# EasyVision-Ton/VMG

Hardware: AMD Instinct MI355X
Metric: LR-frames/s (train: forward+loss+backward+AdamW), VMG-REDS-few_levels 4x SR (higher is better)
Workload: dtype bf16; 1 GPU; VMG-REDS-few_levels train step, per-GPU batch 4x7x3x64x64 -> 4x SR (BASELINE configs[1]); global_batch=4, frames_per_clip=7, parallelism=dp1, launch=eager, recompute_chains=False, fp8_chains=False

## Files before the change

vmg_amd/csrc/conv_igemm.hip:

```cpp
#include <stdlib.h>

#include <type_traits>

#include "common.h"

namespace {

constexpr int MAX_ISRC = 32;
constexpr int CBMAX = 160;

__host__ __device__ constexpr int kstg(int ks) { return ks > 1 ? ks : 2; }
__host__ __device__ constexpr int stage_bytes(int ks, int ntb, int cb) { return kstg(ks) * 4 * ntb * 16 * cb; }
__host__ __device__ constexpr int stage_stride(int ks, int ntb, int cb) { return (stage_bytes(ks, ntb, cb) + 4095) / 4096 * 4096; }
__host__ __device__ inline int stages_of(int ks, int ch) {
  const int nb = (ch / 8 + 3) / 4;
  return ks > 1 ? ks * nb : (nb + 1) / 2;
}

struct ConvK {
  const char* src[MAX_ISRC];
  long long src_ps[MAX_ISRC];
  short src_ch[MAX_ISRC];
  short src_nst[MAX_ISRC];
  int src_pixb[MAX_ISRC];
// ... 371 lines not shown
    for (int sl = 0; sl < nst_s; ++sl, ++gst) {
      asm volatile("s_waitcnt vmcnt(0)" ::: "memory");
      __builtin_amdgcn_s_barrier();
      asm volatile("" ::: "memory");
      if (gst + RING - 1 < nstages) issue_w(gst + RING - 1);

      int boff[KSTG];
      if (KS > 1) {
        const int base = ky * (TWH * pixb) + min(4 * cbk + g, CH - 1) * CB;
#pragma unroll
        for (int j = 0; j < KSTG; ++j) boff[j] = base + j * pixb;
        if (++ky == KS) { ky = 0; ++cbk; }
      } else {
#pragma unroll
        for (int j = 0; j < KSTG; ++j) boff[j] = min(4 * (2 * sl + j) + g, CH - 1) * CB;
      }
      const char* wslot = wbuf + (gst % RING) * SS + g * (COB * CB) + px * CB;

      Frag<T> xf[2][MT], wf[2][NTB];
      auto load_frags = [&](int j, int set) {
#pragma unroll
        for (int mt = 0; mt < MT; ++mt) xf[set][mt].load(pixp[mt] + boff[j]);
#pragma unroll
        for (int ct = 0; ct < NTB; ++ct) wf[set][ct].load(wslot + j * (4 * COB * CB) + ct * 16 * CB);
      };
      load_frags(0, 0);
#pragma unroll
      for (int j = 0; j < KSTG; ++j) {
        if (j + 1 < KSTG) load_frags(j + 1, (j + 1) & 1);
#pragma unroll
        for (int ct = 0; ct < NTB; ++ct)
#pragma unroll
          for (int mt = 0; mt < MT; ++mt) acc[ct][mt] = mma(wf[j & 1][ct], xf[j & 1][mt], acc[ct][mt]);
      }
    }
  }
  asm volatile("s_waitcnt vmcnt(0)" ::: "memory");

#pragma unroll
  for (int mt = 0; mt < MT; ++mt) {
    f32x4 r[NTB];
#pragma unroll
    for (int ct = 0; ct < NTB; ++ct) r[ct] = acc[ct][mt];
    conv_epilogue_row<T, KS, NTB>(a, r, wave * MT + mt, TH, cb, nt_real, n, ty, tx, m0, px, g);
  }
}

template <int NTB>
struct EpiLds {
  static constexpr int COB = NTB * 16, C8 = 2 * NTB, PSTR = COB * 4 + 16, NIT = (16 * C8 + 63) / 64;
  static constexpr int BYTES = 16 * PSTR;
};

template <int KS, int NTB>
__device__ __forceinline__ void conv_epilogue_prefetch8(const ConvK& a, int row, int TH, int cb, int n, int ty, int tx, long long m0, int lane,
                                                        bf16x8 (&pre_res)[EpiLds<NTB>::NIT], bf16x8 (&pre_aux)[EpiLds<NTB>::NIT]) {
  using E = EpiLds<NTB>;
  const bf16* res = reinterpret_cast<const bf16*>(a.res);
  const bf16* aux = reinterpret_cast<const bf16*>(a.aux);
#pragma unroll
  for (int it = 0; it < E::NIT; ++it) {
    const int j = it * 64 + lane, pxi = j / E::C8, c8 = j - pxi * E::C8;
    long long pix;
    const bool valid = conv_row_pixel<KS>(a, row, TH, n, ty, tx, m0, pxi & 15, pix);
    const int co = cb * E::COB + c8 * 8;
    if (j < 16 * E::C8 && valid && co < a.Cout) {
      if (res) pre_res[it] = *reinterpret_cast<const bf16x8*>(res + pix * a.res_ps + co);
      if (aux) pre_aux[it] = *reinterpret_cast<const bf16x8*>(aux + pix * a.aux_ps + co);
    }
  }
}

template <int KS, int NTB>
__device__ __forceinline__ void conv_epilogue_lds8(const ConvK& a, const f32x4 (&acc)[NTB], char* stg, int row, int TH, int cb, int n, int ty, int tx,
                                                   long long m0, int lane, const bf16x8 (&pre_res)[EpiLds<NTB>::NIT],
                                                   const bf16x8 (&pre_aux)[EpiLds<NTB>::NIT], const float* lbias) {
  using E = EpiLds<NTB>;
  const int px = lane & 15, g = lane >> 4;
#pragma unroll
  for (int ct = 0; ct < NTB; ++ct) *reinterpret_cast<f32x4*>(stg + px * E::PSTR + (ct * 16 + g * 4) * 4) = acc[ct];
  bf16* out = reinterpret_cast<bf16*>(a.out);
  bf16* out_pre = reinterpret_cast<bf16*>(a.out_pre);
  const float neg = a.act == VMG_ACT_RELU ? 0.f : (a.act == VMG_ACT_LRELU ? a.slope : 1.f);
#pragma unroll
  for (int it = 0; it < E::NIT; ++it) {
    const int j = it * 64 + lane, pxi = j / E::C8, c8 = j - pxi * E::C8;
    long long pix;
    const bool valid = conv_row_pixel<KS>(a, row, TH, n, ty, tx, m0, pxi & 15, pix);
    const int co = cb * E::COB + c8 * 8;
    if (!(j < 16 * E::C8 && valid && co < a.Cout) || VMG_DBG(a, 8)) continue;
    const f32x4 lo = *reinterpret_cast<const f32x4*>(stg + pxi * E::PSTR + c8 * 32);
    const f32x4 hi = *reinterpret_cast<const f32x4*>(stg + pxi * E::PSTR + c8 * 32 + 16);
    float v[8] = {lo[0], lo[1], lo[2], lo[3], hi[0], hi[1], hi[2], hi[3]};
    if (a.bias) {
      const f32x4 b0 = *reinterpret_cast<const f32x4*>(lbias + c8 * 8), b1 = *reinterpret_cast<const f32x4*>(lbias + c8 * 8 + 4);
#pragma unroll
      for (int r = 0; r < 4; ++r) { v[r] += b0[r]; v[4 + r] += b1[r]; }
    }
    if (out_pre) {
      bf16x8 t;
#pragma unroll
      for (int r = 0; r < 8; ++r) t[r] = (bf16)v[r];
      *reinterpret_cast<bf16x8*>(out_pre + pix * a.out_ps + co) = t;
    }
    if (a.act == VMG_ACT_GELU) {
#pragma unroll
      for (int r = 0; r < 8; ++r) v[r] = gelu_erf(v[r]) * a.alpha;
    } else {
#pragma unroll
      for (int r = 0; r < 8; ++r) v[r] = (v[r] > 0.f ? v[r] : v[r] * neg) * a.alpha;
    }
    if (a.aux) {
#pragma unroll
      for (int r = 0; r < 8; ++r) {
        const float u = (float)pre_aux[it][r];
        v[r] *= a.actgrad == 3 ? gelu_erf_grad(u) : (u > 0.f ? 1.f : (a.actgrad == 2 ? a.slope : 0.f));
      }
    }
    if (a.res) {
#pragma unroll
      for (int r = 0; r < 8; ++r) v[r] += (float)pre_res[it][r];
    }
    bf16x8 t;
#pragma unroll
    for (int r = 0; r < 8; ++r) t[r] = (bf16)v[r];
    *reinterpret_cast<bf16x8*>(out + pix * a.out_ps + co) = t;
  }
}

template <typename T, int KS, int NTB>
__global__ __launch_bounds__(256, (NTB <= 3 ? 3 : 2)) void conv_ksplit_kernel(const ConvK a) {
  constexpr int ES = ElemTraits<T>::ES, CB = ElemTraits<T>::CHUNKB;
  constexpr int TH = 4;
  constexpr int TWH = 16 + KS - 1;
  constexpr int COB = NTB * 16;
  constexpr int SS = stage_stride(KS, NTB, CB);
  constexpr int KSB = 4 * COB * CB;
  extern __shared__ __attribute__((aligned(16))) char smem[];
  char* halo = smem;
  char* zslot = smem + a.halo_bytes;
  float* lbias = reinterpret_cast<float*>(zslot + 16);
  if (VMG_DBG(a, 16)) return;

  const int tid = threadIdx.x, lane = tid & 63;
  const int wave = __builtin_amdgcn_readfirstlane(tid >> 6);
  const int px = lane & 15, g = lane >> 4;
  const int cb = blockIdx.y;
  const int nt_real = min(NTB, (a.Cout - cb * COB + 15) >> 4);
  int n = 0, ty = 0, tx = 0;
  long long m0 = 0;
  if (KS > 1) {
    int bid = xcd_remap(blockIdx.x, gridDim.x, a.dbg);
    tx = bid % a.tiles_x;
    int r = bid / a.tiles_x;
    ty = r % a.tiles_y;
    n = r / a.tiles_y;
  } else {
    m0 = (long long)blockIdx.x * 64;
  }
  conv_stamp(a, wave, 0);
  if (tid < 4) reinterpret_cast<int*>(zslot)[tid] = 0;
  const float bias_r = (tid < COB && a.bias && cb * COB + tid < a.Cout) ? a.bias[cb * COB + tid] : 0.f;

  constexpr bool BF = std::is_same<T, bf16>::value;
  const bool vec8 = BF && a.vec8 != 0;
  bf16x8 pre_res[EpiLds<NTB>::NIT], pre_aux[EpiLds<NTB>::NIT];
  if (vec8) conv_epilogue_prefetch8<KS, NTB>(a, wave, TH, cb, n, ty, tx, m0, lane, pre_res, pre_aux);

  f32x4 acc[NTB][4];
#pragma unroll
  for (int ct = 0; ct < NTB; ++ct)
#pragma unroll
    for (int i = 0; i < 4; ++i) acc[ct][i] = f32x4{0.f, 0.f, 0.f, 0.f};

  const char* wlane = a.wpack + (long long)cb * a.nstages * SS + g * (COB * CB) + px * CB;
  int st0 = 0;
  for (int s = 0; s < a.nsrc; ++s) {
    const int ch = a.src_ch[s], pixb = a.src_pixb[s];
    const int CH = ch >> 3, nb = (CH + 3) >> 2;
    if (s > 0) __syncthreads();
    conv_stamp(a, wave, 1);
    stage_halo<T, KS, 1>(a, s, halo, n, ty, tx, m0, tid);
    if (s == 0 && tid < COB) lbias[tid] = bias_r;
    conv_stamp(a, wave, 3);
    __syncthreads();
    conv_stamp(a, wave, 4);

    const int nks = VMG_DBG(a, 32) ? 0 : (KS > 1 ? 9 * nb : nb);
    const int per = ((nks + 3) / 4 + 2) / 3 * 3;
    const int k0 = wave * per;
    const int rowb = TWH * pixb;
    const char* pixp = halo + px * pixb;
    int rowoff[4];
#pragma unroll
    for (int i = 0; i < 4; ++i) rowoff[i] = ((wave + i) & 3) * rowb;

    Frag<T> wf[3][NTB], xf[3][4];
    struct Cur { int k, cbk, ky, kx; long long woff; };
    auto cur_at = [&](int k) {
      Cur c;
      c.k = k;
      const int kc = min(k, nks - 1);
      if (KS > 1) {
        c.cbk = kc / 9;
        const int tap = kc - 9 * c.cbk;
        c.ky = tap / 3;
        c.kx = tap - 3 * c.ky;
        c.woff = (long long)(st0 + c.cbk * 3 + c.ky) * SS + c.kx * KSB;
      } else {
        c.cbk = kc; c.ky = 0; c.kx = 0;
        c.woff = (long long)(st0 + (kc >> 1)) * SS + (kc & 1) * KSB;
      }
      return c;
    };
    auto advance = [&](Cur& c) {
      ++c.k;
      if (c.k < nks) {
        if (KS > 1) {
          c.woff += KSB;
          if (++c.kx == 3) {
            c.kx = 0;
            c.woff += SS - 3 * KSB;
            if (++c.ky == 3) { c.ky = 0; ++c.cbk; }
          }
        } else {
          c.woff += (c.k & 1) ? KSB : SS - KSB;
          c.cbk = c.k;
        }
      }
    };
    Cur cw = cur_at(k0), cx = cw;
    auto load_w = [&](int set) {
      const char* p = wlane + cw.woff;
#pragma unroll
      for (int ct = 0; ct < NTB; ++ct) wf[set][ct].load(p + ct * 16 * CB);
      advance(cw);
    };
    auto load_x = [&](int set) {
      const bool real = cx.k < nks;
      const int boff = (KS > 1 ? cx.ky * rowb + cx.kx * pixb : 0) + min(4 * cx.cbk + g, CH - 1) * CB;
      const char* base = real ? pixp + boff : zslot;
#pragma unroll
      for (int i = 0; i < 4; ++i) xf[set][i].load(base + (real ? rowoff[i] : 0));
      advance(cx);
    };
    auto mfma_set = [&](int set) {
#pragma unroll
      for (int ct = 0; ct < NTB; ++ct)
#pragma unroll
        for (int i = 0; i < 4; ++i) acc[ct][i] = mma(wf[set][ct], xf[set][i], acc[ct][i]);
    };
    if (nks > 0) {
      load_w(0);
      load_w(1);
      load_x(0);
      for (int i = 0; i < per; i += 3) {
        load_w(2);
        load_x(1);
        mfma_set(0);
        load_w(0);
        load_x(2);
        mfma_set(1);
        load_w(1);
        load_x(0);
        mfma_set(2);
      }
    }
    st0 += a.src_nst[s];
  }

  conv_stamp(a, wave, 5);
  __syncthreads();
  char* scratch = smem;
#pragma unroll
  for (int i = 1; i < 4; ++i) {
    const int q = (wave + i) & 3, j = 4 - i;
    char* dst = scratch + ((q * 3 + (j - 1)) * NTB) * 1024 + lane * 16;
#pragma unroll
    for (int ct = 0; ct < NTB; ++ct) *reinterpret_cast<f32x4*>(dst + ct * 1024) = acc[ct][i];
  }
  __syncthreads();
  f32x4 own[NTB];
#pragma unroll
  for (int ct = 0; ct < NTB; ++ct) own[ct] = acc[ct][0];
#pragma unroll
  for (int j = 1; j < 4; ++j) {
    const char* src = scratch + ((wave * 3 + (j - 1)) * NTB) * 1024 + lane * 16;
#pragma unroll
    for (int ct = 0; ct < NTB; ++ct) {
      const f32x4 t = *reinterpret_cast<const f32x4*>(src + ct * 1024);
      own[ct] += t;
    }
  }
  conv_stamp(a, wave, 6);
  if (vec8) {
    static_assert(EpiLds<NTB>::BYTES <= 3 * NTB * 1024, "epilogue staging patch must fit the wave's own scratch slots");
    conv_epilogue_lds8<KS, NTB>(a, own, scratch + (wave * 3 * NTB) * 1024, wave, TH, cb, n, ty, tx, m0, lane, pre_res, pre_aux, lbias);
  } else {
    conv_epilogue_row<T, KS, NTB, false>(a, own, wave, TH, cb, nt_real, n, ty, tx, m0, px, g);
  }
  conv_stamp(a, wave, 7);
}

template <int NTB, int NS = 1>
__global__ __launch_bounds__(256, NS == 1 ? 2 : 1) void linear_wres_kernel(const ConvK a, int ntiles, int tiles_per_wave) {
  using T = bf16;
  constexpr int KS = 1, CB = 16, NKS = 5, NK = NKS * NS, NDMA = NK;
  constexpr int COB = NTB * 16;
  constexpr int SS = stage_stride(KS, NTB, CB);
  constexpr int KSB = 4 * COB * CB;
  constexpr int XBUF = NDMA * 1024;
  constexpr int WAVE_LDS = 2 * XBUF + ((EpiLds<NTB>::BYTES + 1023) & ~1023);
  extern __shared__ __attribute__((aligned(16))) char smem[];
  const int tid = threadIdx.x, lane = tid & 63;
  const int wave = __builtin_amdgcn_readfirstlane(tid >> 6);
  const int px = lane & 15, g = lane >> 4;
  const int cb = blockIdx.y;
  char* xbuf = smem + wave * WAVE_LDS;
  char* patch = xbuf + 2 * XBUF;
  const int CH = a.src_ch[0] >> 3, nb = (CH + 3) >> 2;
  const int vpp = CH * NS;
  const int pixb = vpp * 16;
  const long long ps_b = a.src_ps[0] * 2;
  const int t0 = (blockIdx.x * 4 + wave) * tiles_per_wave, t1 = min(ntiles, t0 + tiles_per_wave);
  if (t0 >= t1) return;

  Frag<T> wres[NK][NTB];
  {
    const char* wlane = a.wpack + (long long)cb * a.nstages * SS + g * (COB * CB) + px * CB;
#pragma unroll
    for (int k = 0; k < NK; ++k) {
      const int sb = k / NKS, kk = k - sb * NKS;
      const int kc = min(kk, nb - 1);
      const char* p = wlane + (long long)(sb * a.src_nst[0] + (kc >> 1)) * SS + (kc & 1) * KSB;
#pragma unroll
      for (int ct = 0; ct < NTB; ++ct) {
        wres[k][ct].load(p + ct * 16 * CB);
        if (kk >= nb) wres[k][ct].v = bf16x8{0, 0, 0, 0, 0, 0, 0, 0};
      }
    }
  }
  int c_off[NDMA];
  int c_row[NDMA];
#pragma unroll
  for (int i = 0; i < NDMA; ++i) {
    const int L = 64 * i + lane;
    const int r = (int)(((float)L + 0.5f) * (1.0f / (float)vpp));
    c_row[i] = L < 16 * vpp ? r : 16;
    c_off[i] = (int)(r * ps_b) + (L - r * vpp) * 16;
  }
  auto issue = [&](int t, int buf) {
    const long long m0 = (long long)t * 16;
    const char* origin = a.src[0] + m0 * ps_b;
    const long long left = a.M - m0;
#pragma unroll
    for (int i = 0; i < NDMA; ++i) {
      const bool ok = c_row[i] < 16 && c_row[i] < left;
      const char* gp = ok ? origin + c_off[i] : reinterpret_cast<const char*>(&g_conv_zero16);
      __builtin_amdgcn_global_load_lds(GLB_PTR(gp), LDS_PTR(xbuf + buf * XBUF + i * 1024), 16, 0, 0);
    }
  };
  int boff[NK];
#pragma unroll
  for (int k = 0; k < NK; ++k) {
    const int sb = k / NKS, kk = k - sb * NKS;
    boff[k] = px * pixb + (sb * CH + min(4 * kk + g, CH - 1)) * CB;
  }

  issue(t0, 0);
  int buf = 0;
  for (int t = t0; t < t1; ++t, buf ^= 1) {
    const long long m0 = (long long)t * 16;
    bf16x8 pre_res[EpiLds<NTB>::NIT], pre_aux[EpiLds<NTB>::NIT];
    conv_epilogue_prefetch8<KS, NTB>(a, 0, 4, cb, 0, 0, 0, m0, lane, pre_res, pre_aux);
    if (t + 1 < t1) {
      issue(t + 1, buf ^ 1);
      asm volatile("s_waitcnt vmcnt(%0)" ::"n"(NDMA) : "memory");
    } else {
      asm volatile("s_waitcnt vmcnt(0)" ::: "memory");
    }
    f32x4 acc[NTB];
#pragma unroll
    for (int ct = 0; ct < NTB; ++ct) acc[ct] = f32x4{0.f, 0.f, 0.f, 0.f};
    const char* xb = xbuf + buf * XBUF;
#pragma unroll
    for (int k = 0; k < NK; ++k) {
      Frag<T> xf;
      xf.load(xb + boff[k]);
#pragma unroll
      for (int ct = 0; ct < NTB; ++ct) acc[ct] = mma(wres[k][ct], xf, acc[ct]);
    }
    conv_epilogue_lds8<KS, NTB>(a, acc, patch, 0, 4, cb, 0, 0, 0, m0, lane, pre_res, pre_aux, a.bias ? a.bias + cb * COB : nullptr);
  }
}

template <int NCT, int NB, bool FULL>
__global__ __launch_bounds__(512, 1) void conv_wstat_kernel(const ConvK a, int ntiles) {
  using T = bf16;
  constexpr int KS = 3, CB = 16, TH = 8, TWH = 18, THH = 10;
  constexpr int COB = NCT * 16, KSB = 4 * COB * CB;
  constexpr int SS = stage_stride(KS, NCT, CB);
  constexpr int NK = 9 * NB, RW = NCT < 2 ? NCT : 2;
  constexpr int PIXB = 144;
  constexpr int HVEC = THH * TWH * 9, NDMA = (HVEC + 63) / 64, HB = NDMA * 1024;
  constexpr int PSTR = COB * 4 + 16, C8 = 2 * NCT, NITEM = 128 * C8;
  extern __shared__ __attribute__((aligned(16))) char smem[];
  const int tid = threadIdx.x, lane = tid & 63;
  const int wave = __builtin_amdgcn_readfirstlane(tid >> 6);
  const int px = lane & 15, g = lane >> 4;
  const int cb = blockIdx.y;
  const int CH = a.src_ch[0] >> 3;
  constexpr int wbytes = 3 * NB * SS;
  char* wl = smem;
  char* halo = smem + wbytes;
  float* lbias = reinterpret_cast<float*>(halo + 2 * HB);
  char* patch = halo + 2 * HB + COB * 4;

  const int per_xcd = gridDim.x >> 3;
  const int xcd = blockIdx.x & 7, local = blockIdx.x >> 3;
  const int band = (ntiles + 7) >> 3;
  const int band0 = xcd * band, band1 = min(ntiles, band0 + band);
  auto tile_of = [&](int it) { return band0 + it * per_xcd + local; };
  auto barrier = [&]() {
    asm volatile("s_waitcnt lgkmcnt(0)" ::: "memory");
    __builtin_amdgcn_s_barrier();
    asm volatile("" ::: "memory");
  };

  {
    const char* wblk = a.wpack + (long long)cb * wbytes;
    for (int i = tid * 16; i < wbytes; i += 512 * 16) *reinterpret_cast<uint4*>(wl + i) = *reinterpret_cast<const uint4*>(wblk + i);
    for (int i = tid; i < COB; i += 512) lbias[i] = (a.bias && cb * COB + i < a.Cout) ? a.bias[cb * COB + i] : 0.f;
  }

  if (wave >= 4) {
    const int h = wave - 4;
    constexpr int NDH = (NDMA + 3) / 4;
    int lpos[NDH], loff[NDH];
    const long long ps_b = a.src_ps[0] * 2;
#pragma unroll
    for (int k = 0; k < NDH; ++k) {
      const int v = 64 * (h + 4 * k) + lane;
      const int p = v / 9, c = v - p * 9;
      const int hy = p / TWH, hx = p - hy * TWH;
      lpos[k] = (v < HVEC && c < CH) ? (hy << 8) | hx : -1;
      loff[k] = (hy * a.W + hx) * (int)ps_b + c * 16;
    }
    int lfast[NDH];
#pragma unroll
    for (int k = 0; k < NDH; ++k) lfast[k] = lpos[k] >= 0 ? loff[k] : 0;
    auto issue_halo = [&](int t, int buf) {
      const int tx = t % a.tiles_x, r = t / a.tiles_x;
      const int ty = r % a.tiles_y, n = r / a.tiles_y;
      const int y0 = ty * TH - 1, x0 = tx * 16 - 1;
      const char* origin = a.src[0] + (((long long)n * a.H + y0) * a.W + x0) * ps_b;
      char* dst = halo + buf * HB;
      if (VMG_DBG(a, 1)) return;
      if (y0 >= 0 && x0 >= 0 && y0 + THH <= a.H && x0 + TWH <= a.W) {
#pragma unroll
        for (int k = 0; k < NDH; ++k) {
          if (h + 4 * k >= NDMA) break;
          glds16_asm_s(origin, lfast[k], dst + (h + 4 * k) * 1024);
        }
        return;
      }
#pragma unroll
      for (int k = 0; k < NDH; ++k) {
        if (h + 4 * k >= NDMA) break;
        const bool ok = lpos[k] >= 0 && (unsigned)(y0 + (lpos[k] >> 8)) < (unsigned)a.H && (unsigned)(x0 + (lpos[k] & 255)) < (unsigned)a.W;
        const char* gp = ok ? origin + loff[k] : reinterpret_cast<const char*>(&g_conv_zero16);
        glds16_asm(gp, dst + (h + 4 * k) * 1024);
      }
    };
    bf16* out = reinterpret_cast<bf16*>(a.out);
    bf16* out_pre = FULL ? reinterpret_cast<bf16*>(a.out_pre) : nullptr;
    const bf16* res = FULL ? reinterpret_cast<const bf16*>(a.res) : nullptr;
    const bf16* aux = FULL ? reinterpret_cast<const bf16*>(a.aux) : nullptr;
    const float neg = a.act == VMG_ACT_RELU ? 0.f : (a.act == VMG_ACT_LRELU ? a.slope : 1.f);
    int ipos[NCT], ipatch[NCT], ico[NCT];
#pragma unroll
    for (int i = 0; i < NCT; ++i) {
      const int j = 64 * h + lane + 256 * i;
      const int p = j / C8, c8 = j - p * C8;
      ipos[i] = ((p >> 4) << 8) | (p & 15);
      ipatch[i] = p * PSTR + c8 * 32;
      ico[i] = c8 * 8;
    }
    const int nstore = NCT * (out_pre ? 2 : 1);
    int ioff[NCT];
    float ibias[NCT][8];
#pragma unroll
    for (int i = 0; i < NCT; ++i) {
      ioff[i] = (((ipos[i] >> 8) * a.W + (ipos[i] & 255)) * (int)a.out_ps + ico[i]) * 2;
#pragma unroll
      for (int q = 0; q < 8; ++q) ibias[i][q] = (a.bias && cb * COB + ico[i] + q < a.Cout) ? a.bias[cb * COB + ico[i] + q] : 0.f;
    }

    if (tile_of(0) < band1) issue_halo(tile_of(0), 0);
    asm volatile("s_waitcnt vmcnt(0)" ::: "memory");
    for (int it = 0;; ++it) {
      barrier();
      const bool more = tile_of(it) < band1;
      if (more && tile_of(it + 1) < band1) issue_halo(tile_of(it + 1), (it + 1) & 1);
      if (it > 0 && !VMG_DBG(a, 64)) {
        const int t = tile_of(it - 1);
        const int tx = t % a.tiles_x, r = t / a.tiles_x;
        const int ty = r % a.tiles_y, n = r / a.tiles_y;
        const long long pix0 = ((long long)n * a.H + ty * TH) * a.W + tx * 16;
        if (!FULL && ty * TH + TH <= a.H && tx * 16 + 16 <= a.W && cb * COB + COB <= a.Cout && !VMG_DBG(a, 8)) {
          char* obase = reinterpret_cast<char*>(out + pix0 * a.out_ps + cb * COB);
#pragma unroll
          for (int i = 0; i < NCT; ++i) {
            const f32x4 lo = *reinterpret_cast<const f32x4*>(patch + ipatch[i]);
            const f32x4 hi = *reinterpret_cast<const f32x4*>(patch + ipatch[i] + 16);
            float v[8] = {lo[0], lo[1], lo[2], lo[3], hi[0], hi[1], hi[2], hi[3]};
            bf16x8 tq;
#pragma unroll
            for (int q = 0; q < 8; ++q) {
              if (a.bias) v[q] += ibias[i][q];
              v[q] = (v[q] > 0.f ? v[q] : v[q] * neg) * a.alpha;
              tq[q] = (bf16)v[q];
            }
            *reinterpret_cast<bf16x8*>(obase + ioff[i]) = tq;
          }
        } else
#pragma unroll
        for (int i = 0; i < NCT; ++i) {
          const int y = ty * TH + (ipos[i] >> 8), x = tx * 16 + (ipos[i] & 255);
          const int co = cb * COB + ico[i];
          const bool valid = y < a.H && x < a.W && co < a.Cout && !VMG_DBG(a, 8);
          const long long pix = valid ? pix0 + (long long)(ipos[i] >> 8) * a.W + (ipos[i] & 255) : 0;
          const f32x4 lo = *reinterpret_cast<const f32x4*>(patch + ipatch[i]);
          const f32x4 hi = *reinterpret_cast<const f32x4*>(patch + ipatch[i] + 16);
          float v[8] = {lo[0], lo[1], lo[2], lo[3], hi[0], hi[1], hi[2], hi[3]};
          if (a.bias) {
            const f32x4 b0 = *reinterpret_cast<const f32x4*>(lbias + ico[i]), b1 = *reinterpret_cast<const f32x4*>(lbias + ico[i] + 4);
#pragma unroll
            for (int q = 0; q < 4; ++q) { v[q] += b0[q]; v[4 + q] += b1[q]; }
          }
          const int cov = valid ? co : 0;
          if (out_pre) {
            bf16x8 tq;
#pragma unroll
            for (int q = 0; q < 8; ++q) tq[q] = (bf16)v[q];
            bf16* dstp = valid ? out_pre + pix * a.out_ps + co : reinterpret_cast<bf16*>(&g_wstat_trash);
            *reinterpret_cast<bf16x8*>(dstp) = tq;
          }
          if (FULL && a.act == VMG_ACT_GELU) {
#pragma unroll
            for (int q = 0; q < 8; ++q) v[q] = gelu_erf(v[q]) * a.alpha;
          } else {
#pragma unroll
            for (int q = 0; q < 8; ++q) v[q] = (v[q] > 0.f ? v[q] : v[q] * neg) * a.alpha;
          }
          if (aux) {
            const bf16x8 au = *reinterpret_cast<const bf16x8*>(aux + pix * a.aux_ps + cov);
#pragma unroll
            for (int q = 0; q < 8; ++q) {
              const float u = (float)au[q];
              v[q] *= a.actgrad == 3 ? gelu_erf_grad(u) : (u > 0.f ? 1.f : (a.actgrad == 2 ? a.slope : 0.f));
            }
          }
          if (res) {
            const bf16x8 rv = *reinterpret_cast<const bf16x8*>(res + pix * a.res_ps + cov);
#pragma unroll
            for (int q = 0; q < 8; ++q) v[q] += (float)rv[q];
          }
          bf16x8 tq;
#pragma unroll
          for (int q = 0; q < 8; ++q) tq[q] = (bf16)v[q];
          bf16* dst = valid ? out + pix * a.out_ps + co : reinterpret_cast<bf16*>(&g_wstat_trash);
          *reinterpret_cast<bf16x8*>(dst) = tq;
        }
      }
      if (!more) break;
      barrier();
      if (it > 0 && !VMG_DBG(a, 64)) {
        if (nstore == NCT) asm volatile("s_waitcnt vmcnt(%0)" ::"n"(NCT) : "memory");
        else asm volatile("s_waitcnt vmcnt(%0)" ::"n"(2 * NCT) : "memory");
      } else {
        asm volatile("s_waitcnt vmcnt(0)" ::: "memory");
      }
    }
    return;
  }

  barrier();
  Frag<T> wreg[NK][RW];
  const char* wlane = wl + g * (COB * CB) + px * CB;
#pragma unroll
  for (int j = 0; j < NK; ++j)
#pragma unroll
    for (int ct = 0; ct < RW; ++ct) wreg[j][ct].load(wlane + (j / 3) * SS + (j % 3) * KSB + ct * 16 * CB);
  for (int it = 0;; ++it) {
    const int t = tile_of(it);
    if (t >= band1) break;
    const int buf = it & 1;
    f32x4 acc[2][NCT];
#pragma unroll
    for (int mt = 0; mt < 2; ++mt)
#pragma unroll
      for (int ct = 0; ct < NCT; ++ct) acc[mt][ct] = f32x4{0.f, 0.f, 0.f, 0.f};
    const char* hb = halo + buf * HB + ((2 * wave) * TWH + px) * PIXB;
    if (!VMG_DBG(a, 32)) {
      Frag<T> xf[2][2], wf[2][NCT > RW ? NCT - RW : 1];
      auto load_frags = [&](int j, int set) {
        const int cbk = j / 9, tap = j - cbk * 9, ky = tap / 3, kx = tap - ky * 3;
        const char* xc = hb + min(4 * cbk + g, CH - 1) * CB;
#pragma unroll
        for (int mt = 0; mt < 2; ++mt) xf[set][mt].load(xc + ((mt + ky) * TWH + kx) * PIXB);
#pragma unroll
        for (int ct = RW; ct < NCT; ++ct) wf[set][ct - RW].load(wlane + (j / 3) * SS + (j % 3) * KSB + ct * 16 * CB);
      };
      load_frags(0, 0);
#pragma unroll
      for (int j = 0; j < NK; ++j) {
        if (j + 1 < NK) load_frags(j + 1, (j + 1) & 1);
#pragma unroll
        for (int ct = 0; ct < NCT; ++ct)
#pragma unroll
          for (int mt = 0; mt < 2; ++mt) acc[mt][ct] = mma(ct < RW ? wreg[j][ct < RW ? ct : 0] : wf[j & 1][ct >= RW ? ct - RW : 0], xf[j & 1][mt], acc[mt][ct]);
      }
    }
    barrier();
#pragma unroll
    for (int mt = 0; mt < 2; ++mt)
#pragma unroll
      for (int ct = 0; ct < NCT; ++ct) *reinterpret_cast<f32x4*>(patch + ((2 * wave + mt) * 16 + px) * PSTR + (ct * 16 + g * 4) * 4) = acc[mt][ct];
    barrier();
  }
}

template <int NCT>
struct WsGeo {
  static constexpr int COB = NCT * 16;
  static constexpr int KSB = COB * 64;
  static constexpr int STG = 3 * KSB;
  static constexpr int TH = 8, TWH = 18, THH = 10;
  static constexpr int NLW = 3;
  static constexpr int THREADS = (4 + NLW) * 64;
  static constexpr int NIT = EpiLds<NCT>::NIT;
};
__host__ __device__ inline int ws_rem_ksteps(int R) { return R == 0 ? 0 : (R == 1 ? 3 : (R == 2 ? 6 : 9)); }
__host__ __device__ inline int ws_ksteps(int CH) { return 9 * (CH / 4) + ws_rem_ksteps(CH % 4); }
__host__ __device__ inline void ws_slot(int CH, int j, int g, int& tap, int& chunk) {
  const int nfull = CH / 4, R = CH % 4;
  if (j < 9 * nfull) { tap = j % 9; chunk = 4 * (j / 9) + g; return; }
  const int jr = j - 9 * nfull;
  if (R == 1) { tap = 4 * jr + g; chunk = 4 * nfull; }
  else if (R == 2) { tap = 2 * jr + (g >> 1); chunk = 4 * nfull + (g & 1); }
  else { tap = (g == 3) ? -1 : jr; chunk = 4 * nfull + (g == 3 ? 0 : g); }
  if (tap > 8) tap = -1;
}

__device__ __forceinline__ void ws_stamp(const ConvK& a, int wave, int slot) {
#ifdef VMG_DIAG
  if (a.stamps && slot < 32) {
    const unsigned long long t = __builtin_amdgcn_s_memrealtime();
    if ((threadIdx.x & 63) == 0) a.stamps[((size_t)(blockIdx.y * gridDim.x + blockIdx.x) * 8 + wave) * 32 + slot] = t;
  }
#endif
}

template <int NCT>
struct WsItems {
  static constexpr int C8 = 2 * NCT, TOTAL = 128 * C8, THREADS = WsGeo<NCT>::THREADS, NIT = (TOTAL + THREADS - 1) / THREADS;
  static constexpr int PSTR = NCT * 64 + 16;
  __device__ static __forceinline__ void decode(int j, int& pxl, int& c8) {
    pxl = NCT == 9 ? (j * 3641) >> 16 : (NCT == 7 ? (j * 4682) >> 16 : (NCT == 8 ? j >> 4 : (j * 10923) >> 16));
    c8 = j - pxl * C8;
  }
};

template <int NCT>
__global__ __launch_bounds__(WsGeo<NCT>::THREADS, (NCT <= 3 ? 4 : 2)) void conv_ws_kernel(const ConvK a) {
  using G = WsGeo<NCT>;
  using I = WsItems<NCT>;
  using T = bf16;
  constexpr int COB = G::COB, KSB = G::KSB, STG = G::STG;
  static_assert(128 * I::PSTR <= 3 * STG, "the epilogue patch must fit the ring");
  extern __shared__ __attribute__((aligned(16))) char smem[];
  char* halo = smem;
  char* ring = smem + a.halo_bytes;
  const int R = a.ring;
  float* lbias = reinterpret_cast<float*>(ring + R * STG);
  const int tid = threadIdx.x, lane = tid & 63;
  const int wave = __builtin_amdgcn_readfirstlane(tid >> 6);
  const int cb = blockIdx.y;
  const int bid = xcd_remap(blockIdx.x, gridDim.x, 0);
  const int tx = bid % a.tiles_x;
  const int rr = bid / a.tiles_x;
  const int ty = rr % a.tiles_y, n = rr / a.tiles_y;
  const int nstages = a.nstages;
  ws_stamp(a, wave, 0);

  auto issue_halo = [&](int s, int first, int step, auto hidden) {
// ... 721 lines not shown
  using G = WsGeo<NCT>;
  ConvK kk = k;
  kk.ring = NCT <= 3 ? 3 : ((k.halo_bytes + 4 * G::STG + G::COB * 4 <= 160 * 1024) ? 4 : 3);
  const int lds = k.halo_bytes + kk.ring * G::STG + G::COB * 4;
  VMG_CHECK(lds <= 160 * 1024, "conv (weight-streaming): LDS request %d B exceeds 160 KiB", lds);
  auto fn = conv_ws_kernel<NCT>;
  static bool attr_set[VMG_MAX_DEVICES] = {};
  const int dev = vmg_current_device();
  if (!attr_set[dev]) {
    (void)hipFuncSetAttribute(reinterpret_cast<const void*>(fn), hipFuncAttributeMaxDynamicSharedMemorySize, 160 * 1024);
    attr_set[dev] = true;
  }
  const long long nblk = (long long)k.N * k.tiles_y * k.tiles_x;
  VMG_CHECK(nblk > 0 && nblk < (1ll << 31), "conv: bad grid %lld", nblk);
  const bool prof = (k.nsrc == 1 && k.src_ch[0] == k.Cout && (k.Cout == 144 || k.Cout == 112)) && vmg_prof_before(VMG_PROF_CONV3X3, k.M, st);
  hipLaunchKernelGGL(fn, dim3((unsigned)nblk, ncb), dim3(G::THREADS), lds, st, kk);
  if (prof) vmg_prof_after(st);
  VMG_LAUNCH_CHECK();
  return 0;
}

}

#ifdef VMG_DIAG
static unsigned long long* g_conv_stamps = nullptr;
#endif
extern "C" int vmg_conv_debug_stamps(void* buf) {
#ifdef VMG_DIAG
  g_conv_stamps = (unsigned long long*)buf;
  return 0;
#else
  (void)buf;
  vmg_set_error("conv_debug_stamps: this library was built without -DVMG_DIAG (VMG_DIAG=1 python -m vmg_amd.build)");
  return -1;
#endif
}

extern "C" int64_t vmg_conv_pack_bytes(int dtype, int ks, int on, int nsrc, const int* src_ch, int cout_tiles) {
  short xoff[MAX_ISRC], xch[MAX_ISRC];
  const int n = expand_sources(nsrc, nullptr, src_ch, xoff, xch, nullptr);
  if (n < 0 || cout_tiles <= 0 || (ks != 1 && ks != 3 && ks != 7)) return -1;
  int64_t nst = 0;
  for (int s = 0; s < n; ++s) nst += stages_of(ks, xch[s]);
  const int cob = cout_tiles * 16;
  const int ncb = (on + cob - 1) / cob;
  return (int64_t)ncb * nst * stage_stride(ks, cout_tiles, dtype == VMG_BF16 ? 16 : 32);
}

static int fill_pack_std(PackK& p, long long& total, int dtype, const float* w, int O, int I, int ks, int o0, int on, int nsrc, const int* src_off,
                         const int* src_ch, int transpose_flip, int cout_tiles, void* packed) {
  VMG_CHECK(w && packed, "conv_pack: null pointer");
  VMG_CHECK(ks == 1 || ks == 3 || ks == 7, "conv_pack: ks must be 1, 3 or 7");
  VMG_CHECK(dtype == VMG_F32 || dtype == VMG_BF16, "conv_pack: bad dtype");
  VMG_CHECK(nsrc >= 1 && nsrc <= 4, "conv_pack: nsrc must be 1..4");
  VMG_CHECK(!(transpose_flip & 1) || nsrc == 1, "conv_pack: data-gradient packing takes one K slice");
  VMG_CHECK(cout_tiles >= 1 && cout_tiles <= 9, "conv_pack: cout_tiles must be 1..9");
  memset(&p, 0, sizeof(p));
  const int n = expand_sources(nsrc, src_off, src_ch, p.src_off, p.src_ch, nullptr);
  VMG_CHECK(n > 0, "conv_pack: channel slices must be multiples of 8 (and split into <= %d blocks)", MAX_ISRC);
  int st = 0;
  for (int s = 0; s < n; ++s) {
    p.src_st0[s] = (short)st;
    p.src_nst[s] = (short)stages_of(ks, p.src_ch[s]);
    st += p.src_nst[s];
  }
  const int groups = (transpose_flip >> 8) > 1 ? (transpose_flip >> 8) : 1;
  transpose_flip &= 1;
  VMG_CHECK(groups == 1 || (O % groups == 0), "conv_pack: output channels must divide into the groups");
  const int Id = I * groups;
  const int kdim = transpose_flip ? O : Id, odim = transpose_flip ? Id : O;
  for (int s = 0; s < n; ++s) VMG_CHECK(p.src_off[s] >= 0 && p.src_off[s] + p.src_ch[s] <= kdim, "conv_pack: K slice out of range");
  VMG_CHECK(o0 >= 0 && o0 + on <= odim, "conv_pack: output slice out of range");
  p.w = w; p.out = (char*)packed; p.O = O; p.I = I; p.ks = ks; p.o0 = o0; p.on = on; p.nsrc = n;
  p.transpose_flip = transpose_flip; p.groups = groups; p.cob = cout_tiles * 16; p.ncb = (on + p.cob - 1) / p.cob; p.nstages = st;
  const int es = dtype == VMG_BF16 ? 2 : 4;
  p.ss_elems = stage_stride(ks, cout_tiles, es * 8) / es;
  total = (long long)p.ncb * p.nstages * p.ss_elems;
  VMG_CHECK(total < (1ll << 31), "conv_pack: pack of %lld elements (the index arithmetic is 32-bit)", total);
  if (ks == 3 && groups == 1 && (transpose_flip || (uintptr_t)w % 16 == 0) && (transpose_flip || I % 4 == 0)) {
    int nblk = 0;
    for (int s = 0; s < n; ++s) nblk += ((p.src_ch[s] >> 3) + 3) >> 2;
    p.fast3 = 1;
    p.units = (long long)p.ncb * nblk * 4 * p.cob + (long long)p.ncb * p.nstages * (p.ss_elems / 8 - 3 * 4 * p.cob);
  }
  return 0;
}

extern "C" int vmg_conv_pack(int dtype, const float* w, int O, int I, int ks, int o0, int on, int nsrc, const int* src_off,
                             const int* src_ch, int transpose_flip, int cout_tiles, void* packed, void* stream) {
  PackK p;
  long long total = 0;
  const int rc = fill_pack_std(p, total, dtype, w, O, I, ks, o0, on, nsrc, src_off, src_ch, transpose_flip, cout_tiles, packed);
  if (rc) return rc;
  if (p.fast3) {
    const int fb = (int)((p.units + 255) / 256 > 4096 ? 4096 : (p.units + 255) / 256);
    if (dtype == VMG_BF16) hipLaunchKernelGGL((pack3_kernel<bf16, false>), dim3(fb), dim3(256), 0, (hipStream_t)stream, p);
    else hipLaunchKernelGGL((pack3_kernel<float, false>), dim3(fb), dim3(256), 0, (hipStream_t)stream, p);
    VMG_LAUNCH_CHECK();
    return 0;
  }
  const int blocks = (int)((total + 255) / 256 > 4096 ? 4096 : (total + 255) / 256);
  if (dtype == VMG_BF16) hipLaunchKernelGGL(conv_pack_kernel<bf16>, dim3(blocks), dim3(256), 0, (hipStream_t)stream, p);
  else hipLaunchKernelGGL(conv_pack_kernel<float>, dim3(blocks), dim3(256), 0, (hipStream_t)stream, p);
  VMG_LAUNCH_CHECK();
  return 0;
}

static int ws_plan(int nsrc, const int* src_off, const int* src_ch, PackK& p) {
  const int n = expand_sources(nsrc, src_off, src_ch, p.src_off, p.src_ch, nullptr);
  if (n <= 0) return -1;
  int st = 0;
  for (int s = 0; s < n; ++s) {
    p.src_st0[s] = (short)st;
    p.src_nst[s] = (short)(ws_ksteps(p.src_ch[s] >> 3) / 3);
    st += p.src_nst[s];
  }
  p.nsrc = n;
  p.nstages = st;
  return n;
}

extern "C" int64_t vmg_convws_pack_bytes(int on, int nsrc, const int* src_ch, int cout_tiles) {
  PackK p;
  memset(&p, 0, sizeof(p));
  if (cout_tiles <= 0 || cout_tiles > 9 || on <= 0 || nsrc < 1 || nsrc > 4 || ws_plan(nsrc, nullptr, src_ch, p) <= 0) return -1;
  const int cob = cout_tiles * 16;
  return (int64_t)cdiv(on, cob) * p.nstages * 3 * (int64_t)cob * 64;
}

static int fill_pack_ws(PackK& p, long long& total, const float* w, int O, int I, int o0, int on, int nsrc, const int* src_off, const int* src_ch,
                        int transpose_flip, int cout_tiles, void* packed) {
  VMG_CHECK(w && packed, "convws_pack: null pointer");
  VMG_CHECK(cout_tiles == 3 || cout_tiles == 7 || cout_tiles == 8 || cout_tiles == 9, "convws_pack: cout_tiles must be 3, 7, 8 or 9");
  VMG_CHECK(nsrc >= 1 && nsrc <= 4, "convws_pack: nsrc must be 1..4");
  VMG_CHECK(!(transpose_flip & 1) || nsrc == 1, "convws_pack: data-gradient packing takes one K slice");
  const int groups = (transpose_flip >> 8) > 1 ? (transpose_flip >> 8) : 1;
  transpose_flip &= 1;
  VMG_CHECK(groups == 1 || (O % groups == 0), "convws_pack: output channels must divide into the groups");
  memset(&p, 0, sizeof(p));
  VMG_CHECK(ws_plan(nsrc, src_off, src_ch, p) > 0, "convws_pack: channel slices must be multiples of 8 (and split into <= %d blocks)", MAX_ISRC);
  const int Id = I * groups;
  const int kdim = transpose_flip ? O : Id, odim = transpose_flip ? Id : O;
  for (int s = 0; s < p.nsrc; ++s) VMG_CHECK(p.src_off[s] >= 0 && p.src_off[s] + p.src_ch[s] <= kdim, "convws_pack: K slice out of range");
  VMG_CHECK(o0 >= 0 && on > 0 && o0 + on <= odim, "convws_pack: output slice out of range");
  p.w = w; p.out = (char*)packed; p.O = O; p.I = I; p.ks = 3; p.o0 = o0; p.on = on; p.transpose_flip = transpose_flip; p.groups = groups;
  p.cob = cout_tiles * 16; p.ncb = cdiv(on, p.cob);
  total = (long long)p.ncb * p.nstages * 3 * 4 * p.cob * 8;
  VMG_CHECK(total < (1ll << 31), "convws_pack: pack of %lld elements (the index arithmetic is 32-bit)", total);
  bool rem_ok = true;
  for (int s = 0; s < p.nsrc; ++s) rem_ok = rem_ok && (((p.src_ch[s] >> 3) & 3) == 0 || ((p.src_ch[s] >> 3) & 3) == 2);
  if (groups == 1 && rem_ok && (transpose_flip || ((uintptr_t)w % 16 == 0 && I % 4 == 0))) {
    int nblk = 0;
    for (int s = 0; s < p.nsrc; ++s) nblk += ((p.src_ch[s] >> 3) + 3) >> 2;
    p.fast3 = 1;
    p.units = (long long)p.ncb * nblk * 4 * p.cob;
  }
  return 0;
}

extern "C" int vmg_convws_pack(const float* w, int O, int I, int o0, int on, int nsrc, const int* src_off, const int* src_ch,
                               int transpose_flip, int cout_tiles, void* packed, void* stream) {
  PackK p;
  long long total = 0;
  const int rc = fill_pack_ws(p, total, w, O, I, o0, on, nsrc, src_off, src_ch, transpose_flip, cout_tiles, packed);
  if (rc) return rc;
  if (p.fast3) {
    const int fb = (int)((p.units + 255) / 256 > 4096 ? 4096 : (p.units + 255) / 256);
    hipLaunchKernelGGL((pack3_kernel<bf16, true>), dim3(fb), dim3(256), 0, (hipStream_t)stream, p);
    VMG_LAUNCH_CHECK();
    return 0;
  }
  const int blocks = (int)((total + 255) / 256 > 4096 ? 4096 : (total + 255) / 256);
  hipLaunchKernelGGL(convws_pack_kernel, dim3(blocks), dim3(256), 0, (hipStream_t)stream, p);
  VMG_LAUNCH_CHECK();
  return 0;
}

extern "C" int vmg_pack_entry_bytes(void) { return (int)sizeof(PackEntry); }

extern "C" int vmg_pack_entry(void* entry, int kind, int dtype, const float* w, int O, int I, int ks, int o0, int on, int nsrc, const int* src_off,
                              const int* src_ch, int transpose_flip, int cout_tiles, void* packed, int blk0) {
  VMG_CHECK(entry && (kind == 0 || kind == 1) && blk0 >= 0, "pack_entry: bad arguments");
  PackEntry e;
  memset(&e, 0, sizeof(e));
  int rc;
  if (kind == 1) {
    VMG_CHECK(ks == 3 && dtype == VMG_BF16, "pack_entry: the weight-streaming layout is bf16 3x3");
    rc = fill_pack_ws(e.p, e.total, w, O, I, o0, on, nsrc, src_off, src_ch, transpose_flip, cout_tiles, packed);
  } else {
    rc = fill_pack_std(e.p, e.total, dtype, w, O, I, ks, o0, on, nsrc, src_off, src_ch, transpose_flip, cout_tiles, packed);
  }
  if (rc) return rc;
  e.kind = kind; e.dtype = dtype; e.blk0 = blk0;
  long long nb = e.p.fast3 ? (e.p.units + 255) / 256 : (e.total + 256LL * 16 - 1) / (256LL * 16);
  e.nblk = (int)(nb < 1 ? 1 : (nb > 64 ? 64 : nb));
  memcpy(entry, &e, sizeof(e));
  return e.nblk;
}

extern "C" int vmg_pack_run(const void* plan_dev, int n, int total_blocks, void* stream) {
  VMG_CHECK(plan_dev && n > 0 && total_blocks > 0, "pack_run: bad arguments");
  static_assert(sizeof(PackEntry) % 4 == 0, "the block-owner table sits behind the entries");
  hipLaunchKernelGGL(pack_batch_kernel, dim3(total_blocks), dim3(256), 0, (hipStream_t)stream, (const PackEntry*)plan_dev, n);
  VMG_LAUNCH_CHECK();
  return 0;
}

extern "C" int vmg_conv_fwd(const vmg_conv_desc* d, void* stream) {
  VMG_CHECK(d != nullptr, "conv_fwd: null descriptor");
  VMG_CHECK(d->ks == 1 || d->ks == 3 || d->ks == 7, "conv_fwd: ks must be 1, 3 or 7");
  VMG_CHECK(d->dtype == VMG_F32 || d->dtype == VMG_BF16, "conv_fwd: bad dtype");
  VMG_CHECK(d->nsrc >= 1 && d->nsrc <= 4, "conv_fwd: nsrc must be 1..4");
  VMG_CHECK(d->N > 0 && d->H > 0 && d->W > 0 && d->Cout > 0, "conv_fwd: bad shape");
  VMG_CHECK(d->packed && d->out, "conv_fwd: null packed weights / output");
  VMG_CHECK(!d->pixel_shuffle || (d->Cout % 4 == 0), "conv_fwd: pixel_shuffle needs Cout %% 4 == 0");
  VMG_CHECK(!(d->actgrad != 0 && d->aux == nullptr), "conv_fwd: actgrad without aux");
  VMG_CHECK(d->deep == VMG_CONV_GENERAL || d->deep == VMG_CONV_KSPLIT || d->deep == VMG_CONV_WS || d->deep == VMG_CONV_LINEAR_WRES ||
                d->deep == VMG_CONV_WSTAT,
            "conv_fwd: unknown kernel route deep = %d", d->deep);
  const int es = d->dtype == VMG_BF16 ? 2 : 4, cbytes = es * 8;
  ConvK k;
  memset(&k, 0, sizeof(k));
  short xoff[MAX_ISRC];
  int parent[MAX_ISRC];
  const int n = expand_sources(d->nsrc, nullptr, d->src_ch, xoff, k.src_ch, parent);
  VMG_CHECK(n > 0, "conv_fwd: source channel counts must be multiples of 8");
  int mt = d->mt;
  if (d->dtype == VMG_F32) mt = 1;
  const long long M = (long long)d->N * d->H * d->W;
  const int ntb = d->cout_tiles;
  VMG_CHECK(ntb > 0, "conv_fwd: cout_tiles must be positive");
  const int ncb = cdiv(d->Cout, ntb * 16);
  if (d->ks == 7) mt = 1;
  if (mt == 0) mt = 1;
  VMG_CHECK(mt == 1 || mt == 2, "conv_fwd: mt must be 1 or 2");
  const int TH = 4 * mt, TWH = 16 + d->ks - 1, THH = TH + d->ks - 1;
  int kt = 0, halo = 0;
  for (int s = 0; s < n; ++s) {
    const int par = parent[s];
    VMG_CHECK(d->src[par] != nullptr, "conv_fwd: null source %d", par);
    VMG_CHECK(d->src_ps[par] >= d->src_ch[par] && (d->src_ps[par] * es) % 16 == 0, "conv_fwd: source pixel stride must be >= channels and 16-byte aligned");
    VMG_CHECK(((uintptr_t)d->src[par]) % 16 == 0, "conv_fwd: source pointer must be 16-byte aligned");
    k.src[s] = (const char*)d->src[par] + (long long)xoff[s] * es;
    k.src_ps[s] = d->src_ps[par];
    k.src_nst[s] = (short)stages_of(d->ks, k.src_ch[s]);
    k.src_pixb[s] = choose_pixb(k.src_ch[s], es, cbytes);
    kt += k.src_nst[s];
    const int hb = THH * TWH * k.src_pixb[s];
    if (hb > halo) halo = hb;
  }
  k.nsrc = n;
  k.wpack = (const char*)d->packed; k.bias = d->bias;
  k.out = (char*)d->out; k.out_ps = d->out_ps; k.out_pre = (char*)d->out_pre;
  k.res = (const char*)d->res; k.res_ps = d->res_ps; k.aux = (const char*)d->aux; k.aux_ps = d->aux_ps;
  k.N = d->N; k.H = d->H; k.W = d->W; k.Cout = d->Cout; k.M = M;
  k.tiles_x = cdiv(d->W, 16); k.tiles_y = cdiv(d->H, TH);
  k.act = d->act; k.slope = d->slope; k.alpha = d->alpha; k.actgrad = d->aux ? d->actgrad : 0; k.ps = d->pixel_shuffle;
#ifdef VMG_DIAG
  {
    const char* e = getenv("VMG_CONV_DBG");
    k.dbg = e ? atoi(e) : 0;
    k.stamps = g_conv_stamps;
  }
#endif
  {
    auto al = [](const void* p) { return ((uintptr_t)p & 15) == 0; };
    k.vec8 = d->dtype == VMG_BF16 && !d->pixel_shuffle && (d->Cout % 16) == 0 && (d->out_ps % 8) == 0 && al(d->out) &&
             (!d->out_pre || al(d->out_pre)) && (!d->res || ((d->res_ps % 8) == 0 && al(d->res))) &&
             (!d->aux || ((d->aux_ps % 8) == 0 && al(d->aux)));
  }
  k.nstages = kt; k.halo_bytes = (halo + 1023) & ~1023;
  VMG_CHECK(d->out_ps >= (d->pixel_shuffle ? d->Cout / 4 : d->Cout), "conv_fwd: out pixel stride too small");
  hipStream_t st = (hipStream_t)stream;
  if (d->deep == VMG_CONV_WS) {
    VMG_CHECK(d->dtype == VMG_BF16 && d->ks == 3 && k.vec8 && (ntb == 3 || ntb == 7 || ntb == 8 || ntb == 9), "conv_fwd: the weight-streaming kernel is bf16 3x3 with 16-byte aligned rows, cout_tiles 3, 7, 8 or 9");
    for (int s = 0; s < n; ++s) VMG_CHECK(k.src_ch[s] % 16 == 0, "conv_fwd: the weight-streaming kernel takes channel blocks that are multiples of 16 (got %d)", k.src_ch[s]);
    int kt3 = 0, halo3 = 0;
    for (int s = 0; s < n; ++s) {
      k.src_pixb[s] = k.src_ch[s] * 2;
      k.src_nst[s] = (short)(ws_ksteps(k.src_ch[s] >> 3) / 3);
      kt3 += k.src_nst[s];
      const int hb = 10 * 18 * k.src_pixb[s];
      if (hb > halo3) halo3 = hb;
    }
    k.nstages = kt3;
    k.halo_bytes = (halo3 + 1023) & ~1023;
    k.tiles_y = cdiv(d->H, 8);
    return ntb == 9 ? launch_ws<9>(k, ncb, st) : (ntb == 7 ? launch_ws<7>(k, ncb, st) : (ntb == 8 ? launch_ws<8>(k, ncb, st) : launch_ws<3>(k, ncb, st)));
  }
  if (d->deep == VMG_CONV_WSTAT && d->dtype == VMG_BF16 && d->ks == 3 && mt == 1 && k.vec8 && n == 1 && (ntb == 1 || ntb == 3 || ntb == 4) && k.src_ch[0] <= 64 && k.src_ch[0] % 8 == 0 &&
      k.src_ps[0] % 8 == 0 && d->W <= 255 * 16 && (long long)d->W * k.src_ps[0] * 2 * 10 < (1ll << 31)) {
    ConvK kk = k;
    kk.tiles_y = cdiv(d->H, 8);
    const int nb = (k.src_ch[0] / 8 + 3) / 4;
    switch (ntb * 2 + (nb - 1)) {
      case 2: return launch_wstat<1, 1>(kk, ncb, st);
      case 3: return launch_wstat<1, 2>(kk, ncb, st);
      case 6: return launch_wstat<3, 1>(kk, ncb, st);
      case 7: return launch_wstat<3, 2>(kk, ncb, st);
      case 8: return launch_wstat<4, 1>(kk, ncb, st);
      case 9: return launch_wstat<4, 2>(kk, ncb, st);
    }
  }
  if (d->deep == VMG_CONV_LINEAR_WRES && d->dtype == VMG_BF16 && d->ks == 1 && k.vec8 && (ntb == 3 || ntb == 5)) {
    if (n == 1 && k.src_ch[0] <= 160 && k.src_pixb[0] == k.src_ch[0] * 2) return ntb == 3 ? launch_linear_wres<3>(k, ncb, st) : launch_linear_wres<5>(k, ncb, st);
    if (n == 2 && ntb == 3 && d->nsrc == 1 && k.src_ch[0] == k.src_ch[1] && k.src_ch[0] <= 160 && k.src[1] == k.src[0] + k.src_ch[0] * 2 &&
        k.src_nst[0] == k.src_nst[1])
      return launch_linear_wres<3, 2>(k, ncb, st);
  }
  if (d->ks == 7) return d->dtype == VMG_BF16 ? dispatch_ks7<bf16>(k, ntb, ncb, st) : dispatch_ks7<float>(k, ntb, ncb, st);
  if (d->deep == VMG_CONV_KSPLIT) {
    VMG_CHECK(d->dtype == VMG_BF16 && mt == 1, "conv_fwd: the k-split variant is bf16, mt = 1");
    return d->ks == 3 ? dispatch_ksplit<bf16, 3>(k, ntb, ncb, k.halo_bytes, st) : dispatch_ksplit<bf16, 1>(k, ntb, ncb, k.halo_bytes, st);
  }
  if (d->dtype == VMG_BF16) {
    if (d->ks == 3) return mt == 2 ? dispatch_ntb<bf16, 3, 2>(k, ntb, ncb, st) : dispatch_ntb<bf16, 3, 1>(k, ntb, ncb, st);
    return mt == 2 ? dispatch_ntb<bf16, 1, 2>(k, ntb, ncb, st) : dispatch_ntb<bf16, 1, 1>(k, ntb, ncb, st);
  }
  if (d->ks == 3) return dispatch_ntb<float, 3, 1>(k, ntb, ncb, st);
  return dispatch_ntb<float, 1, 1>(k, ntb, ncb, st);
}

static void chain_base(const vmg_chain_desc* c, vmg_conv_desc& d) {
  memset(&d, 0, sizeof(d));
  d.dtype = c->dtype; d.ks = 3; d.N = c->N; d.H = c->H; d.W = c->W; d.Cout = c->C; d.alpha = 1.f;
  d.nsrc = 1; d.src_ps[0] = c->C; d.src_ch[0] = c->C; d.out_ps = c->C; d.cout_tiles = c->cout_tiles; d.deep = c->deep; d.mt = 1;
}

extern "C" int vmg_resblock_chain_fwd(const vmg_chain_desc* c, void* stream) {
  VMG_CHECK(c && c->nblk >= 0 && c->nsrc >= 1 && c->nsrc <= 4 && c->y && c->packed0, "resblock_chain_fwd: bad descriptor");
  VMG_CHECK(c->nblk == 0 || (c->t && c->packed1 && c->packed2 && c->bias1 && c->bias2), "resblock_chain_fwd: null block arrays");
  vmg_conv_desc d;
  chain_base(c, d);
  d.nsrc = c->nsrc;
  for (int s = 0; s < c->nsrc; ++s) { d.src[s] = c->src[s]; d.src_ps[s] = c->src_ps[s]; d.src_ch[s] = c->src_ch[s]; }
  d.packed = c->packed0; d.bias = c->bias0; d.out = c->y[0]; d.act = VMG_ACT_LRELU; d.slope = c->slope0;
  d.cout_tiles = c->cout_tiles0; d.deep = c->deep0;
  int rc = vmg_conv_fwd(&d, stream);
  if (rc) return rc;
  for (int k = 0; k < c->nblk; ++k) {
    chain_base(c, d);
    d.src[0] = c->y[k]; d.packed = c->packed1[k]; d.bias = c->bias1[k]; d.out = c->t[k]; d.act = VMG_ACT_RELU;
    if ((rc = vmg_conv_fwd(&d, stream))) return rc;
    chain_base(c, d);
    d.src[0] = c->t[k]; d.packed = c->packed2[k]; d.bias = c->bias2[k]; d.out = c->y[k + 1]; d.alpha = c->r_scaling;
    d.res = c->y[k]; d.res_ps = c->C;
    if ((rc = vmg_conv_fwd(&d, stream))) return rc;
  }
  return 0;
}

extern "C" int vmg_resblock_chain_bwd(const vmg_chain_desc* c, void* stream) {
  VMG_CHECK(c && c->nblk >= 0 && c->g_y, "resblock_chain_bwd: bad descriptor");
  VMG_CHECK(c->nblk == 0 || (c->t && c->g_t && c->packed1 && c->packed2), "resblock_chain_bwd: null block arrays");
  vmg_conv_desc d;
  for (int k = c->nblk - 1; k >= 0; --k) {
    chain_base(c, d);
    d.src[0] = c->g_y[k + 1]; d.packed = c->packed2[k]; d.out = c->g_t[k]; d.alpha = c->r_scaling; d.aux = c->t[k]; d.aux_ps = c->C; d.actgrad = 1;
    int rc = vmg_conv_fwd(&d, stream);
    if (rc) return rc;
    chain_base(c, d);
    d.src[0] = c->g_t[k]; d.packed = c->packed1[k]; d.out = c->g_y[k]; d.res = c->g_y[k + 1]; d.res_ps = c->C;
    if ((rc = vmg_conv_fwd(&d, stream))) return rc;
  }
  return 0;
}
```

Before: 599.8 LR-frames/s.

## Software-pipeline epilogue operand loads and inline epilogue in linear_wres kernel

Restructures the persistent linear_wres loop so the residual or aux operand for the next tile is loaded alongside that tile's input DMA, with precomputed epilogue indices, bias staged once in LDS, and the epilogue written inline. Wait counts are computed so that stores and operand loads stay in flight across tiles rather than draining every iteration. The loop is unrolled by two with ping-pong operand registers. Cases with both res and aux are excluded from this path, and the change adds register pressure plus fragile hand-coded vmcnt accounting.

Result: no change. 602.8 LR-frames/s (median of 6 runs) (+0.5%).

```diff
diff --git a/vmg_amd/csrc/conv_igemm.hip b/vmg_amd/csrc/conv_igemm.hip
--- a/vmg_amd/csrc/conv_igemm.hip
+++ b/vmg_amd/csrc/conv_igemm.hip
@@ -697,6 +697,8 @@
   conv_stamp(a, wave, 7);
 }
 
+constexpr int vmcnt_imm(int n) { return (n & 15) | (7 << 4) | (15 << 8) | ((n >> 4) << 14); }
+
 template <int NTB, int NS = 1>
 __global__ __launch_bounds__(256, NS == 1 ? 2 : 1) void linear_wres_kernel(const ConvK a, int ntiles, int tiles_per_wave) {
   using T = bf16;
@@ -762,18 +764,50 @@
     boff[k] = px * pixb + (sb * CH + min(4 * kk + g, CH - 1)) * CB;
   }
 
-  issue(t0, 0);
-  int buf = 0;
-  for (int t = t0; t < t1; ++t, buf ^= 1) {
+  using E = EpiLds<NTB>;
+  int e_px[E::NIT], e_co[E::NIT], e_c8[E::NIT];
+  bool e_ok[E::NIT];
+#pragma unroll
+  for (int it = 0; it < E::NIT; ++it) {
+    const int j = it * 64 + lane, pxi = j / E::C8, c8 = j - pxi * E::C8;
+    e_px[it] = pxi & 15;
+    e_c8[it] = c8;
+    e_co[it] = cb * COB + c8 * 8;
+    e_ok[it] = j < 16 * E::C8 && e_co[it] < a.Cout && !VMG_DBG(a, 8);
+  }
+  float* lbias = reinterpret_cast<float*>(patch + E::BYTES);
+  static_assert(E::BYTES + COB * 4 <= ((E::BYTES + 1023) & ~1023), "the bias must fit behind the epilogue patch");
+  if (a.bias && lane < COB / 4) {
+    const int c = cb * COB + 4 * lane;
+    *reinterpret_cast<f32x4*>(lbias + 4 * lane) = c < a.Cout ? *reinterpret_cast<const f32x4*>(a.bias + c) : f32x4{0.f, 0.f, 0.f, 0.f};
+  }
+  const bf16* opnd = reinterpret_cast<const bf16*>(a.aux ? a.aux : a.res);
+  const long long opnd_ps = a.aux ? a.aux_ps : a.res_ps;
+  const bool has_pre = a.out_pre != nullptr;
+  auto load_ops = [&](int t, bf16x8 (&o)[E::NIT]) {
     const long long m0 = (long long)t * 16;
-    bf16x8 pre_res[EpiLds<NTB>::NIT], pre_aux[EpiLds<NTB>::NIT];
-    conv_epilogue_prefetch8<KS, NTB>(a, 0, 4, cb, 0, 0, 0, m0, lane, pre_res, pre_aux);
-    if (t + 1 < t1) {
-      issue(t + 1, buf ^ 1);
-      asm volatile("s_waitcnt vmcnt(%0)" ::"n"(NDMA) : "memory");
-    } else {
-      asm volatile("s_waitcnt vmcnt(0)" ::: "memory");
-    }
+#pragma unroll
+    for (int it = 0; it < E::NIT; ++it) {
+      const long long pix = m0 + e_px[it];
+      const bool ok = e_ok[it] && pix < a.M;
+      const bf16* p = ok ? opnd + pix * opnd_ps + e_co[it] : reinterpret_cast<const bf16*>(&g_conv_zero16);
+      o[it] = *reinterpret_cast<const bf16x8*>(p);
+    }
+  };
+  bf16* out = reinterpret_cast<bf16*>(a.out);
+  bf16* out_pre = reinterpret_cast<bf16*>(a.out_pre);
+  bf16* trash = reinterpret_cast<bf16*>(&g_wstat_trash);
+  const float neg = a.act == VMG_ACT_RELU ? 0.f : (a.act == VMG_ACT_LRELU ? a.slope : 1.f);
+  auto step = [&](int t, int buf, const bf16x8 (&cur)[E::NIT], bf16x8 (&nxt)[E::NIT]) {
+    const int tn = min(t + 1, t1 - 1);
+    issue(tn, buf ^ 1);
+    if (opnd) load_ops(tn, nxt);
+    switch ((opnd != nullptr) + has_pre) {
+      case 0: __builtin_amdgcn_s_waitcnt(vmcnt_imm(NDMA + E::NIT)); break;
+      case 1: __builtin_amdgcn_s_waitcnt(vmcnt_imm(NDMA + 2 * E::NIT)); break;
+      default: __builtin_amdgcn_s_waitcnt(vmcnt_imm(NDMA + 3 * E::NIT)); break;
+    }
+    asm volatile("" ::: "memory");
     f32x4 acc[NTB];
 #pragma unroll
     for (int ct = 0; ct < NTB; ++ct) acc[ct] = f32x4{0.f, 0.f, 0.f, 0.f};
@@ -785,8 +819,62 @@
 #pragma unroll
       for (int ct = 0; ct < NTB; ++ct) acc[ct] = mma(wres[k][ct], xf, acc[ct]);
     }
-    conv_epilogue_lds8<KS, NTB>(a, acc, patch, 0, 4, cb, 0, 0, 0, m0, lane, pre_res, pre_aux, a.bias ? a.bias + cb * COB : nullptr);
-  }
+#pragma unroll
+    for (int ct = 0; ct < NTB; ++ct) *reinterpret_cast<f32x4*>(patch + px * E::PSTR + (ct * 16 + g * 4) * 4) = acc[ct];
+    const long long m0 = (long long)t * 16;
+#pragma unroll
+    for (int it = 0; it < E::NIT; ++it) {
+      const int pxi = e_px[it], c8 = e_c8[it];
+      const long long pix = m0 + pxi;
+      const bool ok = e_ok[it] && pix < a.M;
+      const f32x4 lo = *reinterpret_cast<const f32x4*>(patch + pxi * E::PSTR + c8 * 32);
+      const f32x4 hi = *reinterpret_cast<const f32x4*>(patch + pxi * E::PSTR + c8 * 32 + 16);
+      float v[8] = {lo[0], lo[1], lo[2], lo[3], hi[0], hi[1], hi[2], hi[3]};
+      if (a.bias) {
+        const f32x4 b0 = *reinterpret_cast<const f32x4*>(lbias + c8 * 8), b1 = *reinterpret_cast<const f32x4*>(lbias + c8 * 8 + 4);
+#pragma unroll
+        for (int r = 0; r < 4; ++r) { v[r] += b0[r]; v[4 + r] += b1[r]; }
+      }
+      if (has_pre) {
+        bf16x8 s;
+#pragma unroll
+        for (int r = 0; r < 8; ++r) s[r] = (bf16)v[r];
+        *reinterpret_cast<bf16x8*>(ok ? out_pre + pix * a.out_ps + e_co[it] : trash) = s;
+      }
+      if (a.act == VMG_ACT_GELU) {
+#pragma unroll
+        for (int r = 0; r < 8; ++r) v[r] = gelu_erf(v[r]) * a.alpha;
+      } else {
+#pragma unroll
+        for (int r = 0; r < 8; ++r) v[r] = (v[r] > 0.f ? v[r] : v[r] * neg) * a.alpha;
+      }
+      if (a.aux) {
+#pragma unroll
+        for (int r = 0; r < 8; ++r) {
+          const float u = (float)cur[it][r];
+          v[r] *= a.actgrad == 3 ? gelu_erf_grad(u) : (u > 0.f ? 1.f : (a.actgrad == 2 ? a.slope : 0.f));
+        }
+      } else if (a.res) {
+#pragma unroll
+        for (int r = 0; r < 8; ++r) v[r] += (float)cur[it][r];
+      }
+      bf16x8 s;
+#pragma unroll
+      for (int r = 0; r < 8; ++r) s[r] = (bf16)v[r];
+      *reinterpret_cast<bf16x8*>(ok ? out + pix * a.out_ps + e_co[it] : trash) = s;
+    }
+  };
+
+  bf16x8 op0[E::NIT], op1[E::NIT];
+  issue(t0, 0);
+  if (opnd) load_ops(t0, op0);
+  __builtin_amdgcn_s_waitcnt(vmcnt_imm(0));
+  asm volatile("" ::: "memory");
+  for (int t = t0; t < t1; t += 2) {
+    step(t, 0, op0, op1);
+    if (t + 1 < t1) step(t + 1, 1, op1, op0);
+  }
+  asm volatile("s_waitcnt vmcnt(0)" ::: "memory");
 }
 
 template <int NCT, int NB, bool FULL>
@@ -2114,7 +2202,7 @@
       case 9: return launch_wstat<4, 2>(kk, ncb, st);
     }
   }
-  if (d->deep == VMG_CONV_LINEAR_WRES && d->dtype == VMG_BF16 && d->ks == 1 && k.vec8 && (ntb == 3 || ntb == 5)) {
+  if (d->deep == VMG_CONV_LINEAR_WRES && d->dtype == VMG_BF16 && d->ks == 1 && k.vec8 && (ntb == 3 || ntb == 5) && !(k.res && k.aux)) {
     if (n == 1 && k.src_ch[0] <= 160 && k.src_pixb[0] == k.src_ch[0] * 2) return ntb == 3 ? launch_linear_wres<3>(k, ncb, st) : launch_linear_wres<5>(k, ncb, st);
     if (n == 2 && ntb == 3 && d->nsrc == 1 && k.src_ch[0] == k.src_ch[1] && k.src_ch[0] <= 160 && k.src[1] == k.src[0] + k.src_ch[0] * 2 &&
         k.src_nst[0] == k.src_nst[1])
```
